# Victarry/Image-Generation-models

Hardware: AMD Instinct MI355X
Metric: ddpm_cifar10_32x32_train_images_per_sec (higher is better)
Workload: dtype bf16; 1 GPU; DDPM CIFAR-10 32x32, UNet 128/1-2-4, T=1000 (BASELINE configs[1]): train step B=128/GPU + hipGraph denoise step B=64; per_gpu_batch=128, global_batch=128, parallelism=dp1, step_launch=hipGraph replay, denoise_batch=64, rccl_ranks=1, state_finite=True, matmul=bf16 MFMA, fp32 accumulate

## Files before the change

### image-generation-models_amd/csrc/norm_act.hip

```cpp
#include <stdlib.h>
#include "common.h"

#ifndef MI_GN_UB0
#define MI_GN_UB0 4
#endif
#ifndef MI_GN_PD
#define MI_GN_PD 2
#endif
#ifndef MI_GN_ABL
#define MI_GN_ABL 0
#endif
#ifndef MI_GN_FULL16
#define MI_GN_FULL16 0
#endif
#ifndef MI_GN_WAVES
#define MI_GN_WAVES 4
#endif

namespace {

template <int VEC> struct V;
template <> struct V<4> {
    float v[4];
    __device__ static V load(const float* p) { float4 t = *reinterpret_cast<const float4*>(p); return V{{t.x, t.y, t.z, t.w}}; }
// ... 503 lines not shown
    }
}

int gn_prepare(const MiGnDesc* d, GnArgs& a, int& vec, int& units) {
    if (!d || d->N <= 0 || d->HW <= 0 || d->C <= 0 || d->G <= 0 || d->C % d->G) return -1;
    a.N = d->N; a.HW = d->HW; a.C = d->C; a.G = d->G; a.Cg = d->C / d->G; a.eps = d->eps;
    static const int xcd_env = (int)mi_knob("MI_GN_XCD", 1);
    a.xcd_map = xcd_env;
    a.ldx = d->ldx; a.ldy = d->ldy; a.ldr = d->ldr;
    int cg = a.Cg;
    if (cg & (cg - 1)) return -2;
    if (cg > 128) return -3;
    vec = (cg % 4 == 0) ? 4 : 1;
    if (vec == 1 && cg > 2) return -2;
    int W = cg / vec, PP = 256 / W;
    units = (d->HW + PP - 1) / PP;
    a.vec8_units = (cg % 8 == 0) ? (d->HW + 256 / (cg / 8) - 1) / (256 / (cg / 8)) : 0;
    return 0;
}

struct LnArgs {
    const float* x; const float* g; const float* b; float* y; const float* dy; float* dx; float* dg; float* db;
    int M, C, ldx, ldy, lddy, lddx, accumulate; float eps;
    float* part;
};
constexpr int LN_MAXV = 4;

template <int LPX> __device__ __forceinline__ float group_sum(float v) {
#pragma unroll
    for (int o = LPX / 2; o > 0; o >>= 1) v += __shfl_xor(v, o, 64);
    return v;
}

template <bool Y16, int LPX, int MAXV>
__global__ __launch_bounds__(256) void chan_ln_fwd_kernel(const LnArgs a) {
    MI_PRIO_UP();
    constexpr int PPW = 64 / LPX;
    const int l = threadIdx.x & 63, w = threadIdx.x >> 6, lp = l % LPX;
    const int nq = a.C / 4;
    for (int m0 = (blockIdx.x * 4 + w) * PPW; m0 < a.M; m0 += gridDim.x * 4 * PPW) {
        const int m = min(m0 + l / LPX, a.M - 1);
        const bool live = m0 + l / LPX < a.M;
        const float* xp = a.x + (size_t)m * a.ldx;
        float4 c[MAXV];
        float s = 0.f;
#pragma unroll
// ... 8 lines not shown
            if (lp + LPX * k < nq) {
                float d0 = c[k].x - mean, d1 = c[k].y - mean, d2 = c[k].z - mean, d3 = c[k].w - mean;
                s2 += d0 * d0 + d1 * d1 + d2 * d2 + d3 * d3;
            }
        }
        const float var = group_sum<LPX>(s2) / (float)a.C;
        const float inv = 1.0f / (sqrtf(var) + a.eps);
#pragma unroll
        for (int k = 0; k < MAXV; ++k) {
            int q = lp + LPX * k;
            if (q < nq && live) {
                float4 gg = *reinterpret_cast<const float4*>(a.g + 4 * q);
                float4 bb = *reinterpret_cast<const float4*>(a.b + 4 * q);
                V<4> o;
                o.v[0] = (c[k].x - mean) * inv * gg.x + bb.x; o.v[1] = (c[k].y - mean) * inv * gg.y + bb.y;
                o.v[2] = (c[k].z - mean) * inv * gg.z + bb.z; o.v[3] = (c[k].w - mean) * inv * gg.w + bb.w;
                vstore<4, Y16>(a.y, (size_t)m * a.ldy + 4 * q, o);
            }
        }
    }
}

template <bool DY16, int LPX, int MAXV>
__global__ __launch_bounds__(256) void chan_ln_bwd_kernel(const LnArgs a) {
    MI_PRIO_UP();
    constexpr int PPW = 64 / LPX;
    __shared__ float red[2][4][LPX * MAXV * 4];
    const int l = threadIdx.x & 63, w = threadIdx.x >> 6, lp = l % LPX;
    const int nq = a.C / 4;
    float4 ag[MAXV], ab[MAXV], gg[MAXV];
#pragma unroll
    for (int k = 0; k < MAXV; ++k) {
        ag[k] = ab[k] = make_float4(0.f, 0.f, 0.f, 0.f);
        int q = lp + LPX * k;
        gg[k] = (q < nq) ? *reinterpret_cast<const float4*>(a.g + 4 * q) : make_float4(0.f, 0.f, 0.f, 0.f);
    }
    for (int m0 = (blockIdx.x * 4 + w) * PPW; m0 < a.M; m0 += gridDim.x * 4 * PPW) {
        const int m = min(m0 + l / LPX, a.M - 1);
        const float live = m0 + l / LPX < a.M ? 1.f : 0.f;
        const float* xp = a.x + (size_t)m * a.ldx;
        float4 c[MAXV], d[MAXV];
        float s = 0.f;
#pragma unroll
        for (int k = 0; k < MAXV; ++k) {
            int q = lp + LPX * k;
            if (q < nq) {
                c[k] = *reinterpret_cast<const float4*>(xp + 4 * q);
                const V<4> dv = vload<4, DY16>(a.dy, (size_t)m * a.lddy + 4 * q);
                d[k] = make_float4(dv.v[0] * live, dv.v[1] * live, dv.v[2] * live, dv.v[3] * live);
                s += c[k].x + c[k].y + c[k].z + c[k].w;
            }
        }
        const float mean = group_sum<LPX>(s) / (float)a.C;
        float s2 = 0.f, sh = 0.f, sS = 0.f;
#pragma unroll
        for (int k = 0; k < MAXV; ++k) {
            if (lp + LPX * k < nq) {
                c[k].x -= mean; c[k].y -= mean; c[k].z -= mean; c[k].w -= mean;
                s2 += c[k].x * c[k].x + c[k].y * c[k].y + c[k].z * c[k].z + c[k].w * c[k].w;
                float h0 = d[k].x * gg[k].x, h1 = d[k].y * gg[k].y, h2 = d[k].z * gg[k].z, h3 = d[k].w * gg[k].w;
                sh += h0 + h1 + h2 + h3;
                sS += h0 * c[k].x + h1 * c[k].y + h2 * c[k].z + h3 * c[k].w;
            }
        }
        const float var = group_sum<LPX>(s2) / (float)a.C;
        const float mh = group_sum<LPX>(sh) / (float)a.C;
        const float S = group_sum<LPX>(sS);
        const float sigma = sqrtf(var);
        const float inv = 1.0f / (sigma + a.eps);
        const float k2 = sigma > 0.f ? inv * inv * S / (sigma * (float)a.C) : 0.f;
        float* op = a.dx + (size_t)m * a.lddx;
#pragma unroll
        for (int k = 0; k < MAXV; ++k) {
            int q = lp + LPX * k;
            if (q < nq) {
                float4 o;
                o.x = inv * (d[k].x * gg[k].x - mh) - k2 * c[k].x;
                o.y = inv * (d[k].y * gg[k].y - mh) - k2 * c[k].y;
                o.z = inv * (d[k].z * gg[k].z - mh) - k2 * c[k].z;
                o.w = inv * (d[k].w * gg[k].w - mh) - k2 * c[k].w;
                if (live != 0.f) {
                    if (a.accumulate) {
                        float4 prev = *reinterpret_cast<const float4*>(op + 4 * q);
                        o.x += prev.x; o.y += prev.y; o.z += prev.z; o.w += prev.w;
                    }
                    *reinterpret_cast<float4*>(op + 4 * q) = o;
                }
                ag[k].x += d[k].x * c[k].x * inv; ag[k].y += d[k].y * c[k].y * inv;
                ag[k].z += d[k].z * c[k].z * inv; ag[k].w += d[k].w * c[k].w * inv;
                ab[k].x += d[k].x; ab[k].y += d[k].y; ab[k].z += d[k].z; ab[k].w += d[k].w;
            }
        }
    }
#pragma unroll
    for (int k = 0; k < MAXV; ++k) {
        if constexpr (PPW == 2) {
            ag[k].x += __shfl_xor(ag[k].x, 32, 64); ag[k].y += __shfl_xor(ag[k].y, 32, 64); ag[k].z += __shfl_xor(ag[k].z, 32, 64); ag[k].w += __shfl_xor(ag[k].w, 32, 64);
            ab[k].x += __shfl_xor(ab[k].x, 32, 64); ab[k].y += __shfl_xor(ab[k].y, 32, 64); ab[k].z += __shfl_xor(ab[k].z, 32, 64); ab[k].w += __shfl_xor(ab[k].w, 32, 64);
        }
        int q = lp + LPX * k;
        if (q < nq && l < LPX) {
            red[0][w][4 * q + 0] = ag[k].x; red[0][w][4 * q + 1] = ag[k].y; red[0][w][4 * q + 2] = ag[k].z; red[0][w][4 * q + 3] = ag[k].w;
            red[1][w][4 * q + 0] = ab[k].x; red[1][w][4 * q + 1] = ab[k].y; red[1][w][4 * q + 2] = ab[k].z; red[1][w][4 * q + 3] = ab[k].w;
        }
    }
    __syncthreads();
    for (int c = threadIdx.x; c < a.C; c += 256) {
        float v0 = red[0][0][c] + red[0][1][c] + red[0][2][c] + red[0][3][c];
        float v1 = red[1][0][c] + red[1][1][c] + red[1][2][c] + red[1][3][c];
        if (a.part) {
// ... 339 lines not shown
}
extern "C" int mi_chan_layernorm_fwd_io(int M, int C, const float* x, int ldx, const float* g, const float* b,
                                        float eps, void* y, int ldy, int y16, void* stream) {
    return ln_fwd_go(M, C, x, ldx, g, b, eps, y, ldy, y16, stream);
}
static int ln_fwd_go(int M, int C, const float* x, int ldx, const float* g, const float* b, float eps, void* yv, int ldy, int y16, void* stream) {
    float* y = (float*)yv;
    MI_REQUIRE(M > 0 && C > 0 && C % 4 == 0 && C <= 1024 && ldx % 4 == 0 && ldy % 4 == 0, "C must be a multiple of 4, <= 1024");
    MI_REQUIRE(x && g && b && y, "null argument");
    LnArgs a{};
    a.x = x; a.g = g; a.b = b; a.y = y; a.M = M; a.C = C; a.ldx = ldx; a.ldy = ldy; a.eps = eps;
    const bool half = C <= 128;
    int blocks = (M + (half ? 7 : 3)) / (half ? 8 : 4); if (blocks > 4096) blocks = 4096;
    hipStream_t st = (hipStream_t)stream;
    if (half) { if (y16) hipLaunchKernelGGL((chan_ln_fwd_kernel<true, 32, 1>), dim3(blocks), dim3(256), 0, st, a);
                else     hipLaunchKernelGGL((chan_ln_fwd_kernel<false, 32, 1>), dim3(blocks), dim3(256), 0, st, a); }
    else      { if (y16) hipLaunchKernelGGL((chan_ln_fwd_kernel<true, 64, 4>), dim3(blocks), dim3(256), 0, st, a);
                else     hipLaunchKernelGGL((chan_ln_fwd_kernel<false, 64, 4>), dim3(blocks), dim3(256), 0, st, a); }
    MI_LAUNCH_CHECK();
    return 0;
}

static int ln_bwd_go(int M, int C, const float* x, int ldx, const float* g, float eps, const void* dyv, int lddy, float* dx, int lddx,
                     int accumulate_dx, float* dg, float* db, int dy16, void* stream, float* part = nullptr);
static int ln_bwd_blocks(int M, int C) {
    const bool half = C <= 128;
    static const int capenv = (int)mi_knob("MI_LN_BLOCKS", 0);
    const int cap = capenv ? capenv : 512;
    const int blocks = (M + (half ? 7 : 3)) / (half ? 8 : 4);
    return blocks > cap ? cap : blocks;
}
extern "C" int mi_chan_layernorm_bwd(int M, int C, const float* x, int ldx, const float* g, float eps,
                                     const float* dy, int lddy, float* dx, int lddx, int accumulate_dx,
                                     float* dg, float* db, void* stream) {
    return ln_bwd_go(M, C, x, ldx, g, eps, dy, lddy, dx, lddx, accumulate_dx, dg, db, 0, stream);
}
extern "C" int mi_chan_layernorm_bwd_io(int M, int C, const float* x, int ldx, const float* g, float eps,
                                        const void* dy, int lddy, float* dx, int lddx, int accumulate_dx,
                                        float* dg, float* db, int dy16, void* stream) {
    return ln_bwd_go(M, C, x, ldx, g, eps, dy, lddy, dx, lddx, accumulate_dx, dg, db, dy16, stream);
}
extern "C" int mi_chan_layernorm_bwd_part_rows(int M, int C) { return (M > 0 && C > 0) ? ln_bwd_blocks(M, C) : 0; }
extern "C" int mi_chan_layernorm_bwd_part(int M, int C, const float* x, int ldx, const float* g, float eps,
                                          const void* dy, int lddy, float* dx, int lddx, int accumulate_dx,
                                          float* part, int dy16, void* stream) {
    MI_REQUIRE(part, "null argument");
    return ln_bwd_go(M, C, x, ldx, g, eps, dy, lddy, dx, lddx, accumulate_dx, nullptr, nullptr, dy16, stream, part);
}
static int ln_bwd_go(int M, int C, const float* x, int ldx, const float* g, float eps, const void* dyv, int lddy, float* dx, int lddx,
                     int accumulate_dx, float* dg, float* db, int dy16, void* stream, float* part) {
    const float* dy = (const float*)dyv;
    MI_REQUIRE(M > 0 && C > 0 && C % 4 == 0 && C <= 1024 && ldx % 4 == 0 && lddy % 4 == 0 && lddx % 4 == 0, "C must be a multiple of 4, <= 1024");
    MI_REQUIRE(x && g && dy && dx, "null argument");
    LnArgs a{};
    a.x = x; a.g = g; a.dy = dy; a.dx = dx; a.dg = dg; a.db = db; a.M = M; a.C = C; a.ldx = ldx; a.lddy = lddy;
    a.lddx = lddx; a.accumulate = accumulate_dx; a.eps = eps; a.part = part;
    const bool half = C <= 128;
    const int blocks = ln_bwd_blocks(M, C);
    hipStream_t st = (hipStream_t)stream;
    if (half) { if (dy16) hipLaunchKernelGGL((chan_ln_bwd_kernel<true, 32, 1>), dim3(blocks), dim3(256), 0, st, a);
                else      hipLaunchKernelGGL((chan_ln_bwd_kernel<false, 32, 1>), dim3(blocks), dim3(256), 0, st, a); }
    else      { if (dy16) hipLaunchKernelGGL((chan_ln_bwd_kernel<true, 64, 4>), dim3(blocks), dim3(256), 0, st, a);
                else      hipLaunchKernelGGL((chan_ln_bwd_kernel<false, 64, 4>), dim3(blocks), dim3(256), 0, st, a); }
    MI_LAUNCH_CHECK();
    return 0;
}
```

### image-generation-models_amd/csrc/wgrad1x1_tr.hip

```cpp
#include "tr_common.h"

namespace {

struct W1Args {
    const uint16_t* P; const uint16_t* P2; const void* Q;
    float* ws; float* dW; float* dbias;
    int Ci, Cj, I1, ldp, ldp2, ldq, q32, ni, f32;
    int total, sps, splits, gx, gy, wg0, tile0, xcd_map;
    int gmode;
    int gdy, gdx, lgw, lghw, GH, GW;
};
__device__ __attribute__((aligned(16))) uint32_t g_w1_zero[128];
struct W1Batch { W1Args p[MAXP]; int n; };

constexpr int XSTEP = 64 * 64 * 2;
constexpr int YSTEP = 64 * 128 * 2;
constexpr int YRAW = 64 * 128 * 4;

template <bool Q32, int NI>
__device__ __forceinline__ void wgrad1_body(const W1Args& a, const int wg, uint8_t* lds_raw) {
    constexpr int PF = Q32 ? 2 : 3, RING = PF + 1;
    constexpr int XSLOT = NI * XSTEP;
    constexpr int YOFF = RING * XSLOT;
    constexpr int YSLOT = Q32 ? YRAW : YSTEP;
// ... 391 lines not shown
        MI_REQUIRE(descs[i].mode == descs[0].mode, "one numeric mode per batch");
        MI_REQUIRE(P[i] && Q[i] && dW[i], "null operand");
        MI_REQUIRE(descs[i].I1 == descs[i].Ci || (P2 && P2[i]), "two-source split without P2");
        MI_REQUIRE((((uintptr_t)P[i] | (uintptr_t)Q[i] | (uintptr_t)((P2 && P2[i]) ? P2[i] : P[i])) & 15) == 0, "operands must be 16-byte aligned");
        MI_REQUIRE(!(dbias && dbias[i]) || q_is_fp32[i], "the bias gradient is summed in the fp32 conversion pass (fp32 dY only)");
    }
    w1_shares(n, descs, q_is_fp32, wgs);
    size_t off = 0, lds = 0;
    int wg = 0, tile = 0, nimax = 1, max_splits = 1;
    for (int i = 0; i < n; ++i) {
        W1Args& a = b.p[i];
        w1_plan(&descs[i], a, wgs[i]);
        a.P = (const uint16_t*)P[i]; a.P2 = (const uint16_t*)((P2 && P2[i]) ? P2[i] : P[i]); a.Q = Q[i];
        a.dW = dW[i]; a.dbias = dbias ? dbias[i] : nullptr; a.q32 = q_is_fp32[i] ? 1 : 0; a.f32 = descs[i].mode == 0 ? 1 : 0;
        a.ldp = descs[i].ldp; a.ldp2 = (P2 && P2[i]) ? descs[i].ldp2 : descs[i].ldp; a.ldq = descs[i].ldq;
        a.ws = (float*)workspace + off;
        off += w1_ws_floats(a);
        static const int xcd_env = (int)mi_knob("MI_W1_XCD", 1);
        a.xcd_map = xcd_env && a.gx * a.gy > 1 && a.splits > 1;
        a.wg0 = wg; wg += a.gx * a.gy * a.splits;
        if (a.splits > max_splits) max_splits = a.splits;
        a.tile0 = tile; if (a.splits > 1) { tile += a.gx * a.gy; nimax = a.ni > nimax ? a.ni : nimax; }
        lds = w1_lds(a) > lds ? w1_lds(a) : lds;
    }
    MI_REQUIRE(off == 0 || (workspace && ((uintptr_t)workspace & 15) == 0 && ws_bytes >= off * sizeof(float)),
               "workspace too small (mi_conv1x1_wgrad_tr_batch_workspace)");
    hipStream_t st = (hipStream_t)stream;
    static MiPerDevice once;
    once.run([] {
        (void)hipFuncSetAttribute((const void*)wgrad1x1_tr_kernel, hipFuncAttributeMaxDynamicSharedMemorySize, 160 * 1024);
        (void)hipFuncSetAttribute((const void*)wgrad1x1_f32_kernel, hipFuncAttributeMaxDynamicSharedMemorySize, 160 * 1024); });
    if (g_w1_phase != 2) {
        if (descs[0].mode == 0) hipLaunchKernelGGL(wgrad1x1_f32_kernel, dim3((unsigned)wg), dim3(512), lds, st, b);
        else hipLaunchKernelGGL(wgrad1x1_tr_kernel, dim3((unsigned)wg), dim3(512), lds, st, b);
    }
    if (g_w1_phase != 1 && tile > 0) {
        if (max_splits >= 32) hipLaunchKernelGGL(wgrad1x1_tr_reduce_kernel<8>, dim3(16 * nimax, 4, tile), dim3(256), 0, st, b);
        else hipLaunchKernelGGL(wgrad1x1_tr_reduce_kernel<2>, dim3(4 * nimax, 4, tile), dim3(256), 0, st, b);
    }
    MI_LAUNCH_CHECK();
    return 0;
}

namespace {
bool s2f_ok(const MiWgradDesc* d) {
    if (!d || d->mode != 0 || d->stride != 2 || d->pad != 1 || d->KH != d->KW || (d->KH != 3 && d->KH != 4)) return false;
// ... 84 lines not shown
```

### image-generation-models_amd/src/models/ddpm.py

```python
from __future__ import annotations

import math
import os
from functools import partial
from typing import Dict, List, Optional, Sequence, Tuple

import numpy as np
import torch
from torch import nn

from ..ops import functional as K
from .base import BaseModel, ValidationResult

_HEADS, _DHEAD = 4, 32
_GN_GROUPS = 8


def _mode_id(name: str) -> int:
    if name not in ("fp32", "bf16"):
        raise ValueError(f"compute mode must be 'fp32' or 'bf16', got {name!r}")
    return K.MODE_BF16 if name == "bf16" else K.MODE_FP32


class _Entry:
# ... 122 lines not shown
        self.mid_attn["range"] = span([self.mid_attn["pre"]])
        self.final_range = span(["final_conv."])
        self.time_range = (0, span(["time_mlp."])[1]) if self.with_time else (0, 0)
        col = 0
        for blk in self.res_blocks:
            blk["tcol"] = 0
        for blk, e in zip(self.res_blocks, mlp_w):
            assert e.key == blk["pre"] + "mlp.1.weight"
            blk["tcol"] = col; col += blk["cout"]


class _Node(nn.Module):
    """Anonymous container; the module tree exists only to reproduce the reference's keys."""


class _GradMap:
    def __init__(self):
        self._g: Dict[int, torch.Tensor] = {}
        self._keep: List[torch.Tensor] = []

    def take(self, t: torch.Tensor) -> torch.Tensor:
        return self._g.pop(id(t))

    def add(self, t: torch.Tensor, g: torch.Tensor):
        cur = self._g.get(id(t))
        if cur is None:
            self._g[id(t)] = g; self._keep.append(t)
        else:
            K.axpby(1.0, g, cur, True)

    def target(self, t: torch.Tensor) -> Tuple[torch.Tensor, bool]:
        cur = self._g.get(id(t))
        if cur is not None:
            return cur, True
        buf = torch.empty(t.shape, device=t.device, dtype=t.dtype)
        self._g[id(t)] = buf; self._keep.append(t)
        return buf, False


class _UnetFunction(torch.autograd.Function):

    @staticmethod
    def forward(ctx, x, time, anchor, net):
        y, tape = net._execute(x, time, record=True)
        ctx.net, ctx.tape = net, tape
        ctx.need_dx = x.requires_grad
        return y

    @staticmethod
    def backward(ctx, dy):
        net, tape = ctx.net, ctx.tape
        ctx.tape = None
# ... 6 lines not shown
    def __init__(self, dim, out_dim=None, dim_mults=(1, 2, 4, 8), groups=8, channels=3, with_time_emb=True):
        super().__init__()
        if dim % 8 or dim < 8:
            raise ValueError("dim must be a multiple of 8")
        self.channels = channels
        self.dim = dim
        self.with_time_emb = bool(with_time_emb)
        arch = _Arch(dim, tuple(dim_mults), channels, out_dim, with_time_emb)
        object.__setattr__(self, "_arch", arch)
        self.compute_mode = os.environ.get("MI_DDPM_MODE", "fp32")
        self.block_storage = os.environ.get("MI_DDPM_STORAGE", "bf16")
        self.fuse_gn_conv = os.environ.get("MI_DDPM_FUSE_GN", "auto")
        self.s2_wgrad_tr = K.debug_knob("MI_DDPM_S2_TR", "1") != "0"
        self.final_block16 = K.debug_knob("MI_DDPM_FINAL16", "1") != "0"
        self.ends16 = K.debug_knob("MI_DDPM_ENDS16", "1") != "0"
        self.dual_out = K.debug_knob("MI_DDPM_DUAL_OUT", "1") != "0"
        self.fuse_ln_qkv = K.debug_knob("MI_DDPM_FUSE_LN", "1") != "0"
        self.fuse_ln_qkv_train = K.debug_knob("MI_DDPM_FUSE_LN_TRAIN", "1") != "0"
        self.small_cin_dual = K.debug_knob("MI_DDPM_CIN_DUAL", "1") != "0"
        self.cin_dual_chores = K.debug_knob("MI_DDPM_CIN_CHORES", "1") != "0"
        self.fold_attn = K.debug_knob("MI_DDPM_FOLD_ATTN", "0") == "1"
        self.small_cout_bwd1 = K.debug_knob("MI_DDPM_COUT_BWD1", "1") != "0"
        self.fuse_final = K.debug_knob("MI_DDPM_FUSE_FINAL", "1") != "0"
        self.accumulate_grads = False
        self.grad_ready_hook = None

        flat = torch.zeros(arch.flat_numel)
        for e in arch.entries:
            if e.init == "kaiming":
                w = torch.empty(e.shape)
                nn.init.kaiming_uniform_(w, a=math.sqrt(5))
                e.logical_view(flat).copy_(w)
            elif e.init == "ubias":
                bound = 1 / math.sqrt(e.fan_in) if e.fan_in > 0 else 0
                e.logical_view(flat).copy_(torch.empty(e.shape).uniform_(-bound, bound))
            elif e.init == "one":
                e.logical_view(flat).fill_(1.0)
        object.__setattr__(self, "_flat", flat)
        object.__setattr__(self, "_gflat", None)
        object.__setattr__(self, "_dirty", 0)
        object.__setattr__(self, "_shadow", None)
        object.__setattr__(self, "_shadow_key", None)
        object.__setattr__(self, "_shadow32", None)
        object.__setattr__(self, "_shadow32_key", None)
        object.__setattr__(self, "_anchor", torch.zeros(1, requires_grad=True))
        self._plist: List[Tuple[_Entry, nn.Parameter]] = []
# ... 433 lines not shown
        if record:
            tape.append(("final", h, cF, stF, hF, eps, h_c))
            tape.append(("input", x))
        return eps, tape

    def _backward(self, tape, dy_nchw, need_dx=False):
        d_eps = K.nchw_to_nhwc(dy_nchw)
        return self.backward_nhwc(tape, d_eps, need_dx)

    def backward_nhwc(self, tape, d_eps, need_dx=False):
        A, sv, mode = self._arch, self._sv, _mode_id(self.compute_mode)
        gflat = self.flat_grads
        if not self.accumulate_grads:
            gflat.zero_()
        gv = self._gv
        offs = self._offs
        if mode == K.MODE_BF16:
            wd_sh, wf_sh, wdq_sh, wfq_sh = self._shadows()
        else:
            wdq32_sh, wfq32_sh = self._shadows32()
        G = _GradMap()
        wq = K.WgradQueue(group=int(K.debug_knob("MI_DDPM_WGRAD_GROUP", "8")),
                          group_s2=2 if self.grad_ready_hook is not None else None)
        x_in = tape[-1][1]
        B = x_in.shape[0]
        dtb_all = torch.empty((B, A.mlp_rows), device=x_in.device, dtype=torch.float32)

        def s2_push(dy, inp, pre, k, ci, co, transposed_conv, ihw, ohw, bias):
            big, small = (ohw, ihw) if transposed_conv else (ihw, ohw)
            if dy.dtype != torch.float32 or not K.s2_wgrad_supported(inp.shape[0], k, ci, co, transposed_conv, big, small, mode):
                return None
            x16 = inp if inp.dtype == torch.bfloat16 else K.to_bf16(inp)
            dy16 = K.to_bf16(dy, colsum_out=gv[pre + "bias"] if bias == "colsum" else None, defer=wq)
            ok = wq.push_s2(x16, dy16, gv[pre + "weight"], k=k, Ci=ci, Cj=co, gather_i=not transposed_conv, grid_g=big, grid_d=small,
                            mode=mode)
            assert ok
            return dy16

        def conv_bwd(dy, inp, pre, k, stride=1, pad=0, x2=None, transposed_conv=False, bias="colsum", want_dx=True, winp=None, wx2=None):
            w = sv[pre + "weight"]
            kh, kw, ci, co = w.shape
            ih, iw = inp.shape[1], inp.shape[2]
            oh, ow = dy.shape[1], dy.shape[2]
            winp = inp if winp is None else winp
            wx2 = x2 if wx2 is None else wx2
            dy16 = None
# ... 111 lines not shown
            conv_bwd(dc2, h1, pre + "block2.block.0.", 3, 1, 1, bias=None)
            dh1 = G.take(h1)
            dtb = dtb_all[:, blk["tcol"]:blk["tcol"] + blk["cout"]] if A.with_time else None
            dc1 = K.gn_mish_bwd(c1, st1, sv[pre + "block1.block.1.weight"], sv[pre + "block1.block.1.bias"], dh1,
                                dgamma=gv[pre + "block1.block.1.weight"], dbeta=gv[pre + "block1.block.1.bias"],
                                dtemb=dtb, dbias=gv[pre + "block1.block.0.bias"], out_dtype=c1.dtype)
            conv_bwd(dc1, inp, pre + "block1.block.0.", 3, 1, 1, x2=x2, bias=None, want_dx=want_dx, winp=inp_c, wx2=x2_c)
            if x2 is not None:
                cat = G._g.pop(("cat", id(inp)))
                k1 = inp.shape[3]
                G.add(inp, cat[..., :k1])
                G.add(x2, cat[..., k1:])

        def attn_bwd(rec):
            _, at, inp, ln, qkv, ctx, kstat, ao, out = rec
            pre = at["pre"]
            dout = G.take(out)
            G.add(inp, dout)
            conv_bwd(dout, ao, pre + "fn.fn.to_out.", 1)
            dao = G.take(ao)
            dqkv = K.linattn_bwd(qkv, ctx, kstat, dao, _HEADS)
            conv_bwd(dqkv, ln, pre + "fn.fn.to_qkv.", 1, bias=None)
            dln = G.take(ln)
            wq.flush(kinds=(1,))
            buf, acc = G.target(inp)
            K.chan_layernorm_bwd(inp, sv[pre + "fn.norm.g"], dln, buf, acc, gv[pre + "fn.norm.g"], gv[pre + "fn.norm.b"], defer=wq)

        hook = self.grad_ready_hook
        dx_in = None
        fifo: List[tuple] = []

        def drain():
            while fifo and fifo[0][1] <= wq.flushed:
                hook(*fifo.pop(0)[0])
        wq.on_flush = drain if hook is not None else None
        for rec in reversed(tape):
            kind = rec[0]
            if kind == "input":
                continue
            if hook is not None:
                rng = (A.final_range if kind == "final" else A.time_range if kind == "time" else rec[1]["range"])
            if kind == "final":
                _, h, cF, stF, hF, eps, h_c = rec
                conv_bwd(d_eps, hF, "final_conv.1.", 1)
                dhF = G.take(hF)
                dcF = K.gn_mish_bwd(cF, stF, sv["final_conv.0.block.1.weight"], sv["final_conv.0.block.1.bias"], dhF,
                                    dgamma=gv["final_conv.0.block.1.weight"], dbeta=gv["final_conv.0.block.1.bias"],
                                    dbias=gv["final_conv.0.block.0.bias"], out_dtype=cF.dtype)
                conv_bwd(dcF, h, "final_conv.0.block.0.", 3, 1, 1, bias=None, winp=h_c)
# ... 290 lines not shown
```

### image-generation-models_amd/src/ops/functional.py

```python
from __future__ import annotations

import ctypes as C
import functools
import os
from typing import Optional, Tuple

import torch

from .lib import ROWSUM_MAX, MiConvDesc, MiGnDesc, MiRowSum, MiWgradDesc, check, load_library

MODE_FP32, MODE_BF16 = 0, 1


def debug_knob(name: str, default: str) -> str:
    if os.environ.get("MI_DEBUG_KNOBS") == "1":
        return os.environ.get(name, default)
    return default
PROBE = None


CONV_AUTO = os.environ.get("MI_CONV_AUTO", "1") == "1"


USE_CONV_PW = CONV_AUTO and debug_knob("MI_CONV_PW", "1") == "1"
# ... 1101 lines not shown

def ln_conv1x1(x, g, b, wq, *, Nc, eps=1e-5, bias=None, want_ln=False):
    _need_gpu(x)
    assert x.dtype == torch.float32
    N, H, W, K = x.shape
    y = new_act(N, H, W, Nc, x, torch.bfloat16)
    ln = new_act(N, H, W, K, x, torch.bfloat16) if want_ln else None
    d = MiConvDesc(N=N, IH=H, IW=W, OH=H, OW=W, K=K, Nc=Nc, KH=1, KW=1, stride=1, pad=0, transposed=0, w_kn=0, mode=MODE_BF16, K1=K,
                   ldx=ld_of(x), ldx2=0, ldy=ld_of(y), ldr=0, accumulate=0)
    e0 = _probe_open()
    if want_ln:
        check(load_library().mi_ln_conv1x1_pw_dual(C.byref(d), _p(x), _p(g), _p(b), eps, _p(wq), _p(bias), _p(y), _p(ln), ld_of(ln), _stream()),
              "mi_ln_conv1x1_pw_dual")
    else:
        check(load_library().mi_ln_conv1x1_pw(C.byref(d), _p(x), _p(g), _p(b), eps, _p(wq), _p(bias), _p(y), _stream()), "mi_ln_conv1x1_pw")
    if e0 is not None:
        px, nch = (128 if (K == 128 and N * H * W // 128 >= 512) else 64), K // 128
        g2 = "true" if (px == 64 and N * H * W // 64 < 512) else "false"
        _probe_close(e0, f"ln_conv1x1_pw_kernel<{px}, {nch}, {g2}>", 2.0 * N * H * W * Nc * K, f"N{N} {H}x{W} K{K}->{Nc} fp32 in + LayerNorm",
                     N * H * W * (K * 4 + Nc * 2 + (2 * K if want_ln else 0)) + K * Nc * 2)
    return (y, ln) if want_ln else y


def chan_layernorm_bwd(x, g, dy, dx, accumulate, dg, db, eps=1e-5, defer=None):
    N, H, W, Cc = x.shape
    e0 = _probe_open()
    lib = load_library()
    if defer is not None and dg is not None and db is not None:
        rows = lib.mi_chan_layernorm_bwd_part_rows(N * H * W, Cc)
        part = defer.rows_buffer(x.device, rows * 2 * Cc)
        check(lib.mi_chan_layernorm_bwd_part(N * H * W, Cc, _p(x), ld_of(x), _p(g), eps, _p(dy), ld_of(dy), _p(dx), ld_of(dx),
                                             int(accumulate), _p(part), _b16(dy), _stream()), "mi_chan_layernorm_bwd_part")
        defer.push_rowsum(part, rows, Cc, 2 * Cc, dg)
        defer.push_rowsum(part[Cc:], rows, Cc, 2 * Cc, db)
    else:
        check(lib.mi_chan_layernorm_bwd_io(N * H * W, Cc, _p(x), ld_of(x), _p(g), eps, _p(dy), ld_of(dy), _p(dx),
                                           ld_of(dx), int(accumulate), _p(dg), _p(db), _b16(dy), _stream()),
              "mi_chan_layernorm_bwd")
    if e0 is not None:
        _probe_close(e0, f"chan_ln_bwd_kernel<io{_b16(dy)}>", 0.0, f"M{N * H * W} C{Cc} acc{int(accumulate)}",
                     N * H * W * Cc * (_esz(x) + _esz(dy) + _esz(dx) * (2 if accumulate else 1)))


def small_gemm(ta, tb, A, B, *, bias=None, out=None, accumulate=False, allow_split=False):
    _need_gpu(A)
    I = A.shape[1] if ta else A.shape[0]
    Kc = A.shape[0] if ta else A.shape[1]
    J = B.shape[0] if tb else B.shape[1]
    lib = load_library()
    if (A.dtype != torch.float32 or B.dtype != torch.float32 or A.stride(1) != 1 or B.stride(1) != 1 or
            (A.data_ptr() | B.data_ptr()) & 15 or not lib.mi_small_gemm_supported(int(ta), int(tb), I, J, Kc, A.stride(0), B.stride(0))):
        return None
    if out is None:
        assert not accumulate
        out = torch.empty((I, J), device=A.device, dtype=torch.float32)
    check(lib.mi_small_gemm(int(ta), int(tb), I, J, Kc, _p(A), A.stride(0), _p(B), B.stride(0), _p(bias), _p(out), out.stride(0),
                            int(accumulate), int(allow_split), _stream()), "mi_small_gemm")
    return out


def vq_nearest(z_rows, codebook):
    _need_gpu(z_rows)
    M, D = z_rows.shape
    Kc = codebook.shape[0]
# ... 588 lines not shown
```

### image-generation-models_amd/src/ops/lib.py

```python
from __future__ import annotations

import ctypes as C
import os

_PKG_ROOT = os.path.dirname(os.path.dirname(os.path.dirname(os.path.abspath(__file__))))
_LIB = None


def library_path() -> str:
    return os.environ.get("MI_DDPM_LIB", os.path.join(_PKG_ROOT, "lib", "libmi_ddpm.so"))


class MiConvDesc(C.Structure):
    _fields_ = [(n, C.c_int) for n in (
        "N", "IH", "IW", "OH", "OW", "K", "Nc", "KH", "KW", "stride", "pad", "transposed", "w_kn", "mode",
        "K1", "ldx", "ldx2", "ldy", "ldr", "accumulate")]


class MiWgradDesc(C.Structure):
    _fields_ = [(n, C.c_int) for n in (
        "N", "GH", "GW", "DH", "DW", "Ci", "Cj", "KH", "KW", "stride", "pad", "gather_i", "mode", "I1",
        "ldp", "ldp2", "ldq")]


# ... 124 lines not shown
    "mi_conv3x3_wgrad_supported": [C.POINTER(MiWgradDesc)],
    "mi_conv3x3_wgrad_ws": [C.POINTER(MiWgradDesc), _P, _P, _P, _P, _P, _Z, _P],
    "mi_conv3x3_wgrad_bias": [C.POINTER(MiWgradDesc), _P, _P, _P, _P, _P, _P, _Z, _P],
    "mi_colsum": [_I, _I, _P, _I, _P, _P],
    "mi_gn_mish_fwd": [C.POINTER(MiGnDesc), _P, _P, _P, _P, _I, _P, _P, _P, _P],
    "mi_gn_mish_bwd": [C.POINTER(MiGnDesc), _P, _P, _P, _P, _P, _I, _P, _I, _P, _P, _P, _I, _P, _P],
    "mi_chan_layernorm_fwd": [_I, _I, _P, _I, _P, _P, _F, _P, _I, _P],
    "mi_chan_layernorm_bwd": [_I, _I, _P, _I, _P, _F, _P, _I, _P, _I, _I, _P, _P, _P],
    "mi_linattn_fwd": [_I, _I, _I, _P, _P, _P, _P, _P],
    "mi_linattn_bwd": [_I, _I, _I, _P, _P, _P, _P, _P, _P],
    "mi_vq_partials": [_I],
    "mi_vq_nearest_fwd": [_I, _I, _I, _P, _I, _P, _P, _P, _I, _P, _P],
    "mi_vq_bwd": [_I, _I, _I, _P, _I, _P, _P, _F, _F, _P, _P, _I, _I, _P, _P],
    "mi_vq_scatter_rows": [_I, _I, _I, _P, _I, _P, _P, _P],
    "mi_small_gemm": [_I, _I, _I, _I, _I, _P, _I, _P, _I, _P, _P, _I, _I, _I, _P],
    "mi_small_gemm_supported": [_I, _I, _I, _I, _I, _I, _I],
    "mi_linattn_fwd_io": [_I, _I, _I, _P, _P, _P, _P, _I, _P],
    "mi_linattn_bwd_io": [_I, _I, _I, _P, _P, _P, _P, _P, _I, _P],
    "mi_linattn_fwd_ws": [_I, _I, _I, _P, _P, _P, _P, _I, _P, _Z, _P],
    "mi_linattn_bwd_ws": [_I, _I, _I, _P, _P, _P, _P, _P, _I, _P, _Z, _P],
    "mi_chan_layernorm_fwd_io": [_I, _I, _P, _I, _P, _P, _F, _P, _I, _I, _P],
    "mi_chan_layernorm_bwd_io": [_I, _I, _P, _I, _P, _F, _P, _I, _P, _I, _I, _P, _P, _I, _P],
    "mi_chan_layernorm_bwd_part": [_I, _I, _P, _I, _P, _F, _P, _I, _P, _I, _I, _P, _I, _P],
    "mi_rowsum_batch": [_I, _P, _P],
    "mi_f32_to_bf16_colsum_part": [_Z, _I, _P, _I, _P, _I, _P, _Z, C.POINTER(C.c_int), _P],
    "mi_time_embed": [_I, _I, _P, _P, _P],
    "mi_sample_norm_supported": [_I, _I, _I],
    "mi_sample_norm_fwd": [_I, _I, _I, _P, _P, _P, _P, _P, _F, _P],
    "mi_sample_norm_bwd": [_I, _I, _I, _P, _P, _P, _P, _P, _P, _P, _P, _P],
    "mi_sample_norm_bwd2": [_I, _I, _I, _P, _P, _P, _P, _P, _P, _P, _P, _P],
    "mi_leaky_relu_fwd": [_Z, _P, _P, _F, _P],
    "mi_leaky_relu_bwd": [_Z, _P, _P, _P, _F, _P],
    "mi_tanh_fwd": [_Z, _P, _P, _P],
    "mi_tanh_bwd": [_Z, _P, _P, _P, _P],
    "mi_lerp_rows": [_I, _Z, _P, _P, _P, _P, _P],
    "mi_gp_penalty": [_I, _Z, _P, _P, _P, _F, _P, _P],
    "mi_batchnorm_workspace": [_I],
    "mi_batchnorm_fwd": [_I, _I, _P, _P, _P, _P, _P, _P, _P, _P, _F, _F, _I, _P, _P],
    "mi_batchnorm_bwd": [_I, _I, _P, _P, _P, _P, _P, _P, _P, _P, _P, _P],
    "mi_vae_latent_fwd": [_I, _I, _P, _I, _P, _P, _P, _P],
    "mi_vae_latent_bwd": [_I, _I, _P, _I, _P, _P, _F, _P, _P, _I, _P],
    "mi_adam_tick": [_P, _P],
    "mi_adam_step_dev": [_Z, _P, _P, _P, _P, _P, C.c_double, C.c_double, _F, _F, _P],
    "mi_relu_fwd": [_Z, _P, _P, _P],
    "mi_relu_bwd": [_Z, _P, _P, _P, _I, _P],
    "mi_mish_fwd": [_Z, _P, _P, _P],
# ... 88 lines not shown
```

### include/mi_ddpm.h

```cpp
#ifndef MI_DDPM_H
#define MI_DDPM_H
#include <stddef.h>
#include <stdint.h>

#ifdef __cplusplus
extern "C" {
#endif

#define MI_ABI_VERSION 4
#define MI_MODE_FP32 0
#define MI_MODE_BF16 1

int mi_abi_version(void);
const char* mi_last_error(void);

typedef struct MiConvDesc {
    int N;
    int IH, IW;
    int OH, OW;
    int K;
    int Nc;
    int KH, KW, stride, pad;
    int transposed;
    int w_kn;
// ... 218 lines not shown
                        float* stats, int io, void* stream);
int mi_gn_mish_apply_sums(const MiGnDesc* d, const void* x, const void* sums, const float* gamma, const float* beta, const float* temb,
                          int ldt, const float* residual, void* y, int y_is_bf16, void* y_bf16, int ldy16, float* stats, void* stream);
int mi_gn_stats_coef(const MiGnDesc* d, const void* x, const float* gamma, const float* beta, const float* temb, int ldt,
                     float* stats, float* coef, int x_is_bf16, void* stream);
int mi_gn_mish_bwd_io(const MiGnDesc* d, const void* x, const float* stats, const float* gamma, const float* beta,
                      const void* dout, int lddo, void* dx, int lddx, float* dgamma, float* dbeta, float* dtemb,
                      int ldt, float* dbias, int io, void* stream);

int mi_chan_layernorm_fwd(int M, int C, const float* x, int ldx, const float* g, const float* b,
                          float eps, float* y, int ldy, void* stream);
int mi_chan_layernorm_bwd(int M, int C, const float* x, int ldx, const float* g, float eps,
                          const float* dy, int lddy, float* dx, int lddx, int accumulate_dx,
                          float* dg, float* db, void* stream);
int mi_chan_layernorm_fwd_io(int M, int C, const float* x, int ldx, const float* g, const float* b,
                             float eps, void* y, int ldy, int y16, void* stream);
int mi_chan_layernorm_bwd_io(int M, int C, const float* x, int ldx, const float* g, float eps,
                             const void* dy, int lddy, float* dx, int lddx, int accumulate_dx,
                             float* dg, float* db, int dy16, void* stream);
int mi_chan_layernorm_bwd_part_rows(int M, int C);
int mi_chan_layernorm_bwd_part(int M, int C, const float* x, int ldx, const float* g, float eps,
                               const void* dy, int lddy, float* dx, int lddx, int accumulate_dx,
                               float* part, int dy16, void* stream);

int mi_linattn_fwd(int B, int n, int heads, const float* qkv, float* out, float* ctx,
                   float* kstat, void* stream);
int mi_linattn_bwd(int B, int n, int heads, const float* qkv, const float* ctx,
                   const float* kstat, const float* dout, float* dqkv, void* stream);
int mi_linattn_fwd_io(int B, int n, int heads, const void* qkv, void* out, float* ctx, float* kstat, int b16,
                      void* stream);
int mi_linattn_bwd_io(int B, int n, int heads, const void* qkv, const float* ctx, const float* kstat,
                      const void* dout, void* dqkv, int b16, void* stream);
size_t mi_linattn_workspace(int B, int n, int heads);
int mi_linattn_fwd_ws(int B, int n, int heads, const void* qkv, void* out, float* ctx, float* kstat, int b16,
                      void* workspace, size_t ws_bytes, void* stream);
int mi_linattn_bwd_ws(int B, int n, int heads, const void* qkv, const float* ctx, const float* kstat,
                      const void* dout, void* dqkv, int b16, void* workspace, size_t ws_bytes, void* stream);

int mi_small_gemm(int ta, int tb, int I, int J, int K, const float* A, int lda, const float* B, int ldb,
                  const float* bias, float* C, int ldc, int accumulate, int allow_split, void* stream);
int mi_small_gemm_supported(int ta, int tb, int I, int J, int K, int lda, int ldb);

int mi_vq_partials(int M);
int mi_vq_nearest_fwd(int M, int D, int K, const float* z, int ldz, const float* codebook, int* idx, float* zq, int ldq,
                      float* loss_partial, void* stream);
int mi_vq_bwd(int M, int D, int K, const float* z, int ldz, const float* codebook, const int* idx, float g_vq, float g_commit,
// ... 125 lines not shown
```

Measured before the change: 26800 images/s.

## Write layernorm backward into fresh buffer with residual source to break flush dependency

Adds a variant of the channel layernorm backward that reads the residual gradient from a separate source tensor and writes the sum into a new buffer, replacing the in-place accumulate. In the attention residual block this avoids flushing the pending 1x1 weight-gradient queue before the layernorm backward, because the residual gradient buffer is no longer overwritten while deferred wgrads may still read it. The kernel also hoists the accumulate load earlier for narrow channel counts, makes it branch-free, and raises occupancy hints via launch bounds. The cost is an extra allocation and an unconditional read of the source even when not accumulating.

```diff
diff --git a/image-generation-models_amd/csrc/norm_act.hip b/image-generation-models_amd/csrc/norm_act.hip
--- a/image-generation-models_amd/csrc/norm_act.hip
+++ b/image-generation-models_amd/csrc/norm_act.hip
@@ -549,6 +549,7 @@
 struct LnArgs {
     const float* x; const float* g; const float* b; float* y; const float* dy; float* dx; float* dg; float* db;
     int M, C, ldx, ldy, lddy, lddx, accumulate; float eps;
+    const float* src; int ldsrc;
     float* part;
 };
 constexpr int LN_MAXV = 4;
@@ -603,9 +604,10 @@
 }
 
 template <bool DY16, int LPX, int MAXV>
-__global__ __launch_bounds__(256) void chan_ln_bwd_kernel(const LnArgs a) {
+__global__ __launch_bounds__(256, (DY16 || MAXV == 1) ? 4 : 1) void chan_ln_bwd_kernel(const LnArgs a) {
     MI_PRIO_UP();
     constexpr int PPW = 64 / LPX;
+    constexpr bool PREV_EARLY = MAXV == 1;
     __shared__ float red[2][4][LPX * MAXV * 4];
     const int l = threadIdx.x & 63, w = threadIdx.x >> 6, lp = l % LPX;
     const int nq = a.C / 4;
@@ -620,13 +622,15 @@
         const int m = min(m0 + l / LPX, a.M - 1);
         const float live = m0 + l / LPX < a.M ? 1.f : 0.f;
         const float* xp = a.x + (size_t)m * a.ldx;
-        float4 c[MAXV], d[MAXV];
+        const float* sp = a.src + (size_t)m * a.ldsrc;
+        float4 c[MAXV], d[MAXV], prev[PREV_EARLY ? MAXV : 1];
         float s = 0.f;
 #pragma unroll
         for (int k = 0; k < MAXV; ++k) {
             int q = lp + LPX * k;
             if (q < nq) {
                 c[k] = *reinterpret_cast<const float4*>(xp + 4 * q);
+                if constexpr (PREV_EARLY) prev[k] = *reinterpret_cast<const float4*>(sp + 4 * q);
                 const V<4> dv = vload<4, DY16>(a.dy, (size_t)m * a.lddy + 4 * q);
                 d[k] = make_float4(dv.v[0] * live, dv.v[1] * live, dv.v[2] * live, dv.v[3] * live);
                 s += c[k].x + c[k].y + c[k].z + c[k].w;
@@ -660,13 +664,12 @@
                 o.y = inv * (d[k].y * gg[k].y - mh) - k2 * c[k].y;
                 o.z = inv * (d[k].z * gg[k].z - mh) - k2 * c[k].z;
                 o.w = inv * (d[k].w * gg[k].w - mh) - k2 * c[k].w;
-                if (live != 0.f) {
-                    if (a.accumulate) {
-                        float4 prev = *reinterpret_cast<const float4*>(op + 4 * q);
-                        o.x += prev.x; o.y += prev.y; o.z += prev.z; o.w += prev.w;
-                    }
-                    *reinterpret_cast<float4*>(op + 4 * q) = o;
-                }
+                const bool acc = a.accumulate != 0;
+                float4 pv;
+                if constexpr (PREV_EARLY) pv = prev[k]; else pv = *reinterpret_cast<const float4*>(sp + 4 * q);
+                const float4 t = make_float4(o.x + pv.x, o.y + pv.y, o.z + pv.z, o.w + pv.w);
+                o.x = acc ? t.x : o.x; o.y = acc ? t.y : o.y; o.z = acc ? t.z : o.z; o.w = acc ? t.w : o.w;
+                if (live != 0.f) *reinterpret_cast<float4*>(op + 4 * q) = o;
                 ag[k].x += d[k].x * c[k].x * inv; ag[k].y += d[k].y * c[k].y * inv;
                 ag[k].z += d[k].z * c[k].z * inv; ag[k].w += d[k].w * c[k].w * inv;
                 ab[k].x += d[k].x; ab[k].y += d[k].y; ab[k].z += d[k].z; ab[k].w += d[k].w;
@@ -1052,7 +1055,8 @@
 }
 
 static int ln_bwd_go(int M, int C, const float* x, int ldx, const float* g, float eps, const void* dyv, int lddy, float* dx, int lddx,
-                     int accumulate_dx, float* dg, float* db, int dy16, void* stream, float* part = nullptr);
+                     int accumulate_dx, float* dg, float* db, int dy16, void* stream, float* part = nullptr,
+                     const float* src = nullptr, int ldsrc = 0, bool src_given = false);
 static int ln_bwd_blocks(int M, int C) {
     const bool half = C <= 128;
     static const int capenv = (int)mi_knob("MI_LN_BLOCKS", 0);
@@ -1077,14 +1081,34 @@
     MI_REQUIRE(part, "null argument");
     return ln_bwd_go(M, C, x, ldx, g, eps, dy, lddy, dx, lddx, accumulate_dx, nullptr, nullptr, dy16, stream, part);
 }
+extern "C" int mi_chan_layernorm_bwd_src(int M, int C, const float* x, int ldx, const float* g, float eps,
+                                         const void* dy, int lddy, const float* src, int ldsrc, float* dx, int lddx,
+                                         float* dg, float* db, int dy16, void* stream) {
+    return ln_bwd_go(M, C, x, ldx, g, eps, dy, lddy, dx, lddx, 0, dg, db, dy16, stream, nullptr, src, ldsrc, true);
+}
+extern "C" int mi_chan_layernorm_bwd_src_part(int M, int C, const float* x, int ldx, const float* g, float eps,
+                                              const void* dy, int lddy, const float* src, int ldsrc, float* dx, int lddx,
+                                              float* part, int dy16, void* stream) {
+    MI_REQUIRE(part, "null argument");
+    return ln_bwd_go(M, C, x, ldx, g, eps, dy, lddy, dx, lddx, 0, nullptr, nullptr, dy16, stream, part, src, ldsrc, true);
+}
 static int ln_bwd_go(int M, int C, const float* x, int ldx, const float* g, float eps, const void* dyv, int lddy, float* dx, int lddx,
-                     int accumulate_dx, float* dg, float* db, int dy16, void* stream, float* part) {
+                     int accumulate_dx, float* dg, float* db, int dy16, void* stream, float* part, const float* src, int ldsrc, bool src_given) {
     const float* dy = (const float*)dyv;
     MI_REQUIRE(M > 0 && C > 0 && C % 4 == 0 && C <= 1024 && ldx % 4 == 0 && lddy % 4 == 0 && lddx % 4 == 0, "C must be a multiple of 4, <= 1024");
     MI_REQUIRE(x && g && dy && dx, "null argument");
+    if (src_given) accumulate_dx = src != nullptr;
+    else { src = accumulate_dx ? dx : nullptr; ldsrc = lddx; }
+    if (!src) { src = dx; ldsrc = lddx; }
+    MI_REQUIRE(ldsrc % 4 == 0 && ((uintptr_t)src & 15) == 0, "src rows must be 16-byte aligned");
+    MI_REQUIRE(src != dx || ldsrc == lddx, "in place: one pitch");
+    if (src != dx) {
+        const uintptr_t s0 = (uintptr_t)src, s1 = s0 + ((size_t)(M - 1) * ldsrc + C) * 4, d0 = (uintptr_t)dx, d1 = d0 + ((size_t)(M - 1) * lddx + C) * 4;
+        MI_REQUIRE(!accumulate_dx || s1 <= d0 || d1 <= s0, "src must be dx itself or not overlap it");
+    }
     LnArgs a{};
     a.x = x; a.g = g; a.dy = dy; a.dx = dx; a.dg = dg; a.db = db; a.M = M; a.C = C; a.ldx = ldx; a.lddy = lddy;
-    a.lddx = lddx; a.accumulate = accumulate_dx; a.eps = eps; a.part = part;
+    a.lddx = lddx; a.accumulate = accumulate_dx; a.eps = eps; a.part = part; a.src = src; a.ldsrc = ldsrc;
     const bool half = C <= 128;
     const int blocks = ln_bwd_blocks(M, C);
     hipStream_t st = (hipStream_t)stream;
diff --git a/image-generation-models_amd/csrc/wgrad1x1_tr.hip b/image-generation-models_amd/csrc/wgrad1x1_tr.hip
--- a/image-generation-models_amd/csrc/wgrad1x1_tr.hip
+++ b/image-generation-models_amd/csrc/wgrad1x1_tr.hip
@@ -437,6 +437,15 @@
         if (a.splits > max_splits) max_splits = a.splits;
         a.tile0 = tile; if (a.splits > 1) { tile += a.gx * a.gy; nimax = a.ni > nimax ? a.ni : nimax; }
         lds = w1_lds(a) > lds ? w1_lds(a) : lds;
+    }
+    static const int dbg = (int)mi_knob("MI_WTR_DEBUG", 0);
+    if (dbg) {
+        fprintf(stderr, "[wgrad1x1_tr] %d layers, %d workgroups\n", n, wg);
+        for (int i = 0; i < n; ++i) {
+            const W1Args& a = b.p[i];
+            fprintf(stderr, "   Ci%-4d Cj%-4d dY %s tiles %2d x splits %3d (steps/slice %3d of %4d): %.2f MB per workgroup\n", a.Ci, a.Cj, a.q32 ? "fp32" : "bf16",
+                    a.gx * a.gy, a.splits, a.sps, a.total, 64.0 * a.sps * (a.ni * 64 * 2 + 128 * (a.q32 ? 4 : 2)) / 1e6);
+        }
     }
     MI_REQUIRE(off == 0 || (workspace && ((uintptr_t)workspace & 15) == 0 && ws_bytes >= off * sizeof(float)),
                "workspace too small (mi_conv1x1_wgrad_tr_batch_workspace)");
diff --git a/image-generation-models_amd/src/models/ddpm.py b/image-generation-models_amd/src/models/ddpm.py
--- a/image-generation-models_amd/src/models/ddpm.py
+++ b/image-generation-models_amd/src/models/ddpm.py
@@ -168,12 +168,20 @@
     def take(self, t: torch.Tensor) -> torch.Tensor:
         return self._g.pop(id(t))
 
+    def peek(self, t: torch.Tensor):
+        return self._g.get(id(t))
+
     def add(self, t: torch.Tensor, g: torch.Tensor):
         cur = self._g.get(id(t))
         if cur is None:
             self._g[id(t)] = g; self._keep.append(t)
         else:
             K.axpby(1.0, g, cur, True)
+
+    def replace(self, t: torch.Tensor, g: torch.Tensor) -> torch.Tensor:
+        old = self._g[id(t)]
+        self._g[id(t)] = g
+        return old
 
     def target(self, t: torch.Tensor) -> Tuple[torch.Tensor, bool]:
         cur = self._g.get(id(t))
@@ -226,6 +234,7 @@
         self.fold_attn = K.debug_knob("MI_DDPM_FOLD_ATTN", "0") == "1"
         self.small_cout_bwd1 = K.debug_knob("MI_DDPM_COUT_BWD1", "1") != "0"
         self.fuse_final = K.debug_knob("MI_DDPM_FUSE_FINAL", "1") != "0"
+        self.ln_bwd_inplace = K.debug_knob("MI_DDPM_LN_BWD_INPLACE", "0") == "1"
         self.accumulate_grads = False
         self.grad_ready_hook = None
 
@@ -705,6 +714,7 @@
         G = _GradMap()
         wq = K.WgradQueue(group=int(K.debug_knob("MI_DDPM_WGRAD_GROUP", "8")),
                           group_s2=2 if self.grad_ready_hook is not None else None)
+        ln_inplace = self.grad_ready_hook is not None or self.ln_bwd_inplace
         x_in = tape[-1][1]
         B = x_in.shape[0]
         dtb_all = torch.empty((B, A.mlp_rows), device=x_in.device, dtype=torch.float32)
@@ -862,9 +872,14 @@
             dqkv = K.linattn_bwd(qkv, ctx, kstat, dao, _HEADS)
             conv_bwd(dqkv, ln, pre + "fn.fn.to_qkv.", 1, bias=None)
             dln = G.take(ln)
-            wq.flush(kinds=(1,))
-            buf, acc = G.target(inp)
-            K.chan_layernorm_bwd(inp, sv[pre + "fn.norm.g"], dln, buf, acc, gv[pre + "fn.norm.g"], gv[pre + "fn.norm.b"], defer=wq)
+            if ln_inplace or G.peek(inp) is not dout:
+                wq.flush(kinds=(1,))
+                buf, acc = G.target(inp)
+                K.chan_layernorm_bwd(inp, sv[pre + "fn.norm.g"], dln, buf, acc, gv[pre + "fn.norm.g"], gv[pre + "fn.norm.b"], defer=wq)
+                return
+            buf = torch.empty(dout.shape, device=dout.device, dtype=torch.float32)
+            K.chan_layernorm_bwd(inp, sv[pre + "fn.norm.g"], dln, buf, True, gv[pre + "fn.norm.g"], gv[pre + "fn.norm.b"], defer=wq, src=dout)
+            G.replace(inp, buf)
 
         hook = self.grad_ready_hook
         dx_in = None
diff --git a/image-generation-models_amd/src/ops/functional.py b/image-generation-models_amd/src/ops/functional.py
--- a/image-generation-models_amd/src/ops/functional.py
+++ b/image-generation-models_amd/src/ops/functional.py
@@ -1147,24 +1147,38 @@
     return (y, ln) if want_ln else y
 
 
-def chan_layernorm_bwd(x, g, dy, dx, accumulate, dg, db, eps=1e-5, defer=None):
+def chan_layernorm_bwd(x, g, dy, dx, accumulate, dg, db, eps=1e-5, defer=None, src=None):
     N, H, W, Cc = x.shape
     e0 = _probe_open()
     lib = load_library()
-    if defer is not None and dg is not None and db is not None:
-        rows = lib.mi_chan_layernorm_bwd_part_rows(N * H * W, Cc)
+    M = N * H * W
+    if src is not None:
+        assert src.dtype == torch.float32 and tuple(src.shape) == tuple(x.shape)
+        if defer is not None and dg is not None and db is not None:
+            rows = lib.mi_chan_layernorm_bwd_part_rows(M, Cc)
+            part = defer.rows_buffer(x.device, rows * 2 * Cc)
+            check(lib.mi_chan_layernorm_bwd_src_part(M, Cc, _p(x), ld_of(x), _p(g), eps, _p(dy), ld_of(dy), _p(src), ld_of(src), _p(dx), ld_of(dx),
+                                                     _p(part), _b16(dy), _stream()), "mi_chan_layernorm_bwd_src_part")
+            defer.push_rowsum(part, rows, Cc, 2 * Cc, dg)
+            defer.push_rowsum(part[Cc:], rows, Cc, 2 * Cc, db)
+        else:
+            check(lib.mi_chan_layernorm_bwd_src(M, Cc, _p(x), ld_of(x), _p(g), eps, _p(dy), ld_of(dy), _p(src), ld_of(src), _p(dx), ld_of(dx),
+                                                _p(dg), _p(db), _b16(dy), _stream()), "mi_chan_layernorm_bwd_src")
+        accumulate = True
+    elif defer is not None and dg is not None and db is not None:
+        rows = lib.mi_chan_layernorm_bwd_part_rows(M, Cc)
         part = defer.rows_buffer(x.device, rows * 2 * Cc)
-        check(lib.mi_chan_layernorm_bwd_part(N * H * W, Cc, _p(x), ld_of(x), _p(g), eps, _p(dy), ld_of(dy), _p(dx), ld_of(dx),
+        check(lib.mi_chan_layernorm_bwd_part(M, Cc, _p(x), ld_of(x), _p(g), eps, _p(dy), ld_of(dy), _p(dx), ld_of(dx),
                                              int(accumulate), _p(part), _b16(dy), _stream()), "mi_chan_layernorm_bwd_part")
         defer.push_rowsum(part, rows, Cc, 2 * Cc, dg)
         defer.push_rowsum(part[Cc:], rows, Cc, 2 * Cc, db)
     else:
-        check(lib.mi_chan_layernorm_bwd_io(N * H * W, Cc, _p(x), ld_of(x), _p(g), eps, _p(dy), ld_of(dy), _p(dx),
+        check(lib.mi_chan_layernorm_bwd_io(M, Cc, _p(x), ld_of(x), _p(g), eps, _p(dy), ld_of(dy), _p(dx),
                                            ld_of(dx), int(accumulate), _p(dg), _p(db), _b16(dy), _stream()),
               "mi_chan_layernorm_bwd")
     if e0 is not None:
-        _probe_close(e0, f"chan_ln_bwd_kernel<io{_b16(dy)}>", 0.0, f"M{N * H * W} C{Cc} acc{int(accumulate)}",
-                     N * H * W * Cc * (_esz(x) + _esz(dy) + _esz(dx) * (2 if accumulate else 1)))
+        _probe_close(e0, f"chan_ln_bwd_kernel<io{_b16(dy)}>", 0.0, f"M{M} C{Cc} acc{int(accumulate)}{' src' if src is not None else ''}",
+                     M * Cc * (_esz(x) + _esz(dy) + _esz(dx) * (2 if accumulate else 1)))
 
 
 def small_gemm(ta, tb, A, B, *, bias=None, out=None, accumulate=False, allow_split=False):
diff --git a/image-generation-models_amd/src/ops/lib.py b/image-generation-models_amd/src/ops/lib.py
--- a/image-generation-models_amd/src/ops/lib.py
+++ b/image-generation-models_amd/src/ops/lib.py
@@ -170,6 +170,8 @@
     "mi_chan_layernorm_fwd_io": [_I, _I, _P, _I, _P, _P, _F, _P, _I, _I, _P],
     "mi_chan_layernorm_bwd_io": [_I, _I, _P, _I, _P, _F, _P, _I, _P, _I, _I, _P, _P, _I, _P],
     "mi_chan_layernorm_bwd_part": [_I, _I, _P, _I, _P, _F, _P, _I, _P, _I, _I, _P, _I, _P],
+    "mi_chan_layernorm_bwd_src": [_I, _I, _P, _I, _P, _F, _P, _I, _P, _I, _P, _I, _P, _P, _I, _P],
+    "mi_chan_layernorm_bwd_src_part": [_I, _I, _P, _I, _P, _F, _P, _I, _P, _I, _P, _I, _P, _I, _P],
     "mi_rowsum_batch": [_I, _P, _P],
     "mi_f32_to_bf16_colsum_part": [_Z, _I, _P, _I, _P, _I, _P, _Z, C.POINTER(C.c_int), _P],
     "mi_time_embed": [_I, _I, _P, _P, _P],
diff --git a/include/mi_ddpm.h b/include/mi_ddpm.h
--- a/include/mi_ddpm.h
+++ b/include/mi_ddpm.h
@@ -264,6 +264,12 @@
 int mi_chan_layernorm_bwd_part(int M, int C, const float* x, int ldx, const float* g, float eps,
                                const void* dy, int lddy, float* dx, int lddx, int accumulate_dx,
                                float* part, int dy16, void* stream);
+int mi_chan_layernorm_bwd_src(int M, int C, const float* x, int ldx, const float* g, float eps,
+                              const void* dy, int lddy, const float* src, int ldsrc, float* dx, int lddx,
+                              float* dg, float* db, int dy16, void* stream);
+int mi_chan_layernorm_bwd_src_part(int M, int C, const float* x, int ldx, const float* g, float eps,
+                                   const void* dy, int lddy, const float* src, int ldsrc, float* dx, int lddx,
+                                   float* part, int dy16, void* stream);
 
 int mi_linattn_fwd(int B, int n, int heads, const float* qkv, float* out, float* ctx,
                    float* kstat, void* stream);
```

New measurement: 27060 images/s (median of 6 runs). About the same (+1.0%).
